# recursiveGecko/Formula-VAD

Hardware: AMD Instinct MI355X
Metric: 20ms audio frames/sec end-to-end VAD pipeline (higher is better)
Workload: dtype f32

## Files before the change

### formula-vad_amd/csrc/engine.cpp

```cpp
#include <algorithm>
#include <cctype>
#include <cmath>
#include <cstdio>
#include <cstdlib>
#include <cstring>
#include <atomic>
#include <mutex>
#include <thread>

#include "internal.h"

#ifndef FVAD_DIAG
#define FVAD_DIAG 0
#endif

namespace fvad {

int set_err(const fvad_ctx* ctx, int code, const std::string& msg)
{
    if (ctx) ctx->err = msg;
    return code;
}
int hip_fail(const fvad_ctx* ctx, hipError_t e, const char* what)
{
// ... 120 lines not shown
#endif
        tn.ws2_variant = (int)c;
    } else if (name == "ws2_waits") {
        long c = 0;
        if (!unset && (!to_long(c) || c < 0 || c > 0x7FFFFFFFL)) return FVAD_ERR_INVALID_ARGUMENT;
        tn.ws2_waits = (unsigned)c;
    } else if (name == "ws2_calibrate") {
        bool on = false;
        if (!to_bool(on)) return FVAD_ERR_INVALID_ARGUMENT;
        for (unsigned& w : tn.ws2_waits_cal) w = 0;
        if (on) { const int rc = calibrate_ws2_waits(ctx); if (rc) return rc; }
    } else if (name == "gru_lat_tiles") {
        long c = 0;
        if (!unset && (!to_long(c) || c < 1 || c > 3)) return FVAD_ERR_INVALID_ARGUMENT;
        tn.gru_lat_tiles = (int)c;
    } else if (name == "k4_plain_loads") { if (!to_bool(tn.k4_plain_loads)) return FVAD_ERR_INVALID_ARGUMENT; }
    else if (name == "no_pipeline") { if (!to_bool(tn.no_pipeline)) return FVAD_ERR_INVALID_ARGUMENT; }
    else if (name == "trace_run") { if (!to_bool(tn.trace_run)) return FVAD_ERR_INVALID_ARGUMENT; }
    else if (name == "run_groups") {
        if (!unset) {
            int sum = 0, n = 0, cur = 0;
            bool digit = false;
            for (char c : v + ",") {
                if (c >= '0' && c <= '9') { cur = cur * 10 + (c - '0'); digit = true; if (cur > 16) return FVAD_ERR_INVALID_ARGUMENT; }
                else if (c == ',' && digit && cur > 0) { sum += cur; ++n; cur = 0; digit = false; }
                else return FVAD_ERR_INVALID_ARGUMENT;
            }
            if (sum != 16 || n > 7) return FVAD_ERR_INVALID_ARGUMENT;
        }
        tn.run_groups = v;
// ... 659 lines not shown
```

### formula-vad_amd/csrc/internal.h

```cpp
#pragma once
#include <hip/hip_runtime.h>

#include <cstdint>
#include <map>
#include <memory>
#include <string>
#include <vector>

#include "../../include/fvad.h"
#include "kernels.h"

namespace fvad {

void hann_window_periodic(float* result, size_t n);
void hann_window_symmetric(float* result, size_t n);
float window_norm_factor(const float* w, size_t n);
void nsnet2_window(float* w320);
void make_twiddles(int n, std::vector<float>& out);
void make_super_twiddles(int ncfft, std::vector<float>& out);

struct HostWeights {
    int n_bins = 0, n_fc1 = 0, n_hidden = 0, n_fc2 = 0, n_fc3 = 0;
    std::vector<float> fc1_w, fc1_b, gru1_w, gru1_r, gru1_b, gru2_w, gru2_r, gru2_b, fc2_w, fc2_b,
        fc3_w, fc3_b, fc4_w, fc4_b;
// ... 111 lines not shown
    bool trace_run = false;
    std::string run_groups;
    int gru_lat_tiles = 0;
    bool k4_plain_loads = false;
    int copy_threads = 8;
    bool trace_kernels = false;
    bool reproducible = false;
    int vad_lane_map = 0;
    int vad_size_order = 0;
    int vad_chain = 0;
    int vad_avgs = 0;
    unsigned long long vad_avgs_max_bytes = 16ull << 30;
    int vad_trigger = 0;
    unsigned long long vad_trigger_max_bytes = 4ull << 30;
    int vad_seg_cap = 0;
    int ws2_variant = 0;
    unsigned ws2_waits = 0;
    unsigned ws2_waits_cal[4] = {0, 0, 0, 0};
    unsigned long long ws_spin_ticks = 0ull;
    bool ws_spin_auto = true;
};

}

struct fvad_ctx {
    int device = 0;
    int n_cu = 256;
    hipStream_t stream = nullptr;
    hipStream_t part_stream = nullptr;
    hipEvent_t part_ev = nullptr;
// ... 36 lines not shown
    } while (0)

int upload_model(fvad_ctx* ctx);
int dev_alloc(fvad_ctx* ctx, float** p, size_t n_floats, bool zero);
int grow(fvad_ctx* ctx, float** p, size_t* cap, size_t need);
void free_workspace_nn(Workspace& ws);
long planned_max_chunks(const fvad_ctx* ctx, long total, long max_chunks);
void plan_launches(const fvad_ctx* ctx, long total, long max_chunks, std::vector<long>& plan);
int ensure_workspace_plan(fvad_ctx* ctx, const std::vector<long>& plan);
long padded_batch(const fvad_ctx* ctx, long n, int T, int skip);
int nn_math_effective(const fvad_ctx* ctx);
int ensure_workspace(fvad_ctx* ctx, long n_chunks, int T, int skip, long n_last = 0);
int ensure_gru_ws(fvad_ctx* ctx);
int get_vad_plan(fvad_ctx* ctx, size_t n, VadFftPlan* out, bool force_generic = false);
bool fvad_fft_size_ok(size_t n);
int run_nn(fvad_ctx* ctx, long n_chunks_pad, int T, int skip, long n_real = 0);
int calibrate_ws2_waits(fvad_ctx* ctx);

struct LaneJob {
    const float* d_in;
    float* d_den;
    size_t n_chunks;
    LaneCarry* carry[2];
    int cur;
    float* d_rms;
    float* h_spec = nullptr;
    float* h_feat = nullptr;
    const int16_t* d_in16 = nullptr;
    int16_t* d_den16 = nullptr;
};
int run_chunks(fvad_ctx* ctx, std::vector<LaneJob>& jobs, long max_chunks, ChunkDesc* capture_descs = nullptr,
// ... 5 lines not shown
```

### formula-vad_amd/csrc/kernels.h

```cpp
#pragma once
#include <hip/hip_runtime.h>
#include <stddef.h>
#include <stdint.h>

#include "../../include/fvad.h"

enum { FVAD_ACT_NONE = 0, FVAD_ACT_RELU = 1, FVAD_ACT_SIGMOID = 2 };

constexpr int kNFft = 320;
constexpr int kNHop = 160;
constexpr int kFramesPerChunk = 50;
constexpr int kWarmupRows = 4;
constexpr int kRowsPerChunk = kFramesPerChunk + kWarmupRows;
constexpr int kNBins = 161;
constexpr int kFeatStride = 176;
constexpr int kDown = 3;
constexpr int kChunk48 = kFramesPerChunk * kNHop * kDown;
constexpr int kVadFft = 1024;
constexpr int kVadFftMax = 16384;

struct LaneCarry {
    float in_tail[kNHop * kDown];
    float feat_tail[kWarmupRows * kNBins];
    float ola_tail[kNHop];
// ... 39 lines not shown
};

int fvad_launch_panel_gemm(const float* A, int lda, const float* Wfrag, const float* bias, float* C,
                           int ldc, long rows, int nt, int n_blocks, int S_steps, int act,
                           int map_T, int map_skip, hipStream_t stream, int n_valid_tiles = 0,
                           const unsigned* guard = nullptr);
struct GemmRowMap {
    int n_rows = 0, L = 0, in_T = 0, in_t0 = 0, out_T = 0, out_t0 = 0;
};
int fvad_launch_panel_gemm_s_rows(const float* A, int lda, const float* Wfrag, const float* bias, float* C, int ldc,
                                  GemmRowMap rm, int nt, int n_blocks, int S_steps, int act, hipStream_t stream,
                                  int n_valid_tiles = 0, const unsigned* guard = nullptr);
int fvad_launch_panel_gemm_s(const float* A, int lda, const float* Wfrag, const float* bias, float* C, int ldc,
                             long rows, int nt, int n_blocks, int S_steps, int act, int map_T, int map_skip,
                             hipStream_t stream, int n_valid_tiles = 0, const unsigned* guard = nullptr);
int fvad_launch_panel_gemm3(const float* A, int lda, const float* Wfrag, const float* bias, float* C,
                            int ldc, long rows, int nt, int n_blocks, int S_steps, int K, int act,
                            int n_valid_tiles, int map_T, int map_skip, int n_wg, hipStream_t stream);
int fvad_launch_panel_gemm_h3(const float* A, int in_ts, int a_ld, const float* Wfrag, const float* bias, float* C,
                              int out, int c_ld, int seq_T, long row_tiles, int nt, int n_blocks, int K, int act,
                              int n_valid_tiles, int map_T, int map_skip, float sx, float sw, float out_sx, int n_wg,
                              hipStream_t stream);
int fvad_launch_gru_rec_h3(const float* gi, const float* Rfrag, const float* bR, float* hsplit,
                           long n_seq_pad, int T, int waves, float sx, float sw, hipStream_t stream);
int fvad_launch_gru_ws2_fallback(float* gi, const float* feat, const float* W1frag_nt2, const float* bG1, const float* R1frag, const float* bR1,
                                 const float* W2frag_nt2, const float* bW2, const float* R2frag, const float* bR2, float* h1, float* h2,
                                 long n_seq_pad, int T, unsigned* sync, unsigned long long* fallbacks, hipStream_t stream,
                                 int zero_at = 0, int zero_n = 0);
int fvad_launch_gru_lat(const float* gi, const float* R2frag, const float* bR, float* hout,
                        long n_seq_pad, int T, const unsigned* guard, int tile_major, hipStream_t stream, int row_tiles = 1);
void fvad_launch_zero_words(unsigned* p, int n, hipStream_t stream);
void fvad_launch_count_word(unsigned long long* counter, const unsigned* word, hipStream_t stream);
bool fvad_gru_ws_shape(long n_seq_pad, int n_cu, int* RT, int* G);
// ... 5 lines not shown
size_t fvad_gru_ws2_exchange_floats(long n_seq_pad);
bool fvad_gru_ws2_gi1_in_kernel(long n_seq_pad, int T, int n_cu, int variant);
bool fvad_gru_ws2_ok(long n_seq_pad, int T, int n_cu, int variant);
const char* fvad_gru_ws2_kernel_name(long n_seq_pad, int T, int n_cu, int variant);
int fvad_launch_gru_ws2(const float* gi1, const float* feat, const float* W1frag, const float* bG1, const float* R1frag, const float* bR1,
                        const float* W2frag, const float* bW2, const float* R2frag, const float* bR2, float* hout2, float* hx,
                        unsigned* flags, unsigned* err, long n_seq_pad, int T, int n_cu, unsigned long long spin_ticks, int variant,
                        unsigned waits, hipStream_t stream, unsigned* lsync = nullptr);
constexpr int kWs2LocalWords = 336;
bool fvad_gru_ws2_local_layer1(long n_seq_pad, int T, int n_cu, int variant);
int fvad_gru_ws2_wait_class(long n_seq_pad, int T, int n_cu, int variant);
unsigned fvad_gru_ws2_builtin_waits(int wait_class, bool local_layer1 = false);
int fvad_launch_gru_gen(const float* gi, int gi_ld, const float* R2frag, const float* bR, float* hout, int h_ld,
                        long n_seq_pad, int T, int J, hipStream_t stream);
int fvad_launch_gru_rec3(const float* gi, const float* R2frag, const float* bR, float* hout,
                         long n_seq_pad, int T, int waves, hipStream_t stream, float* hs3 = nullptr);
int fvad_launch_panel_gemm_b3(const float* A, int in_ts, int a_ld, const float* Wfrag, const float* bias, float* C,
                              int out, int c_ld, int seq_T, long row_tiles, int nt, int n_blocks, int K, int act,
                              int n_valid_tiles, int map_T, int map_skip, int n_wg, hipStream_t stream);

void fvad_launch_stft(const ChunkDesc* descs, int n_chunks, FftTables tb, float* feat,
                      float* spec, hipStream_t stream, int parts = 1);
void fvad_launch_istft(const ChunkDesc* descs, int n_chunks, FftTables tb, const float* spec,
                       const float* gains, int gains_rows_per_chunk, int gains_row0,
                       hipStream_t stream, int parts = 1);
void fvad_launch_vadfft(const float* den, long n_frames, VadFftPlan pl, int min_bin, int max_bin,
                        float* band_sum, float* bins_or_null, hipStream_t stream);
int fvad_launch_vadfft_jobs(const VadFftJob* jobs, int n_jobs, long max_frames, VadFftPlan pl,
                            int min_bin, int max_bin, hipStream_t stream, int any_bins, int n_cu, int plain_loads = 0);
constexpr int kVadBandsPerLaunch = 256;
struct VadBandSet {
// ... 162 lines not shown
```

### formula-vad_amd/csrc/kernels_nn.hip

```cpp

#include <hip/hip_runtime.h>
#include <stdint.h>
#include <type_traits>

#include "kernels.h"

#include "nn_device.h"

__device__ __forceinline__ float act_sigmoid(float x) { return 1.0f / (1.0f + expf(-x)); }

template <int NT, int ACT, int WAVES>
__global__ __launch_bounds__(WAVES * 64) void panel_gemm_kernel(
    const float* __restrict__ A, int lda, const float* __restrict__ Wfrag,
    const float* __restrict__ bias, float* __restrict__ C, int ldc, int S_steps, int row_map_T,
    int row_map_skip, int n_valid_tiles, const unsigned* guard)
{
    __shared__ __attribute__((aligned(16))) float slab[2][NT * 256];
    if (guard && *guard == 0) return;

    const int tid = threadIdx.x;
    const int lane = tid & 63;
    const int wave = tid >> 6;
    const int m = lane & 15;
    const int q = lane >> 4;
// ... 268 lines not shown
    }
};
template <int N> struct StaticFor<N, N> {
    template <class F> static __device__ __forceinline__ void run(F&&) {}
};

template <int OFF> __device__ __forceinline__ void lds_read_b128(f32x4& dst, unsigned addr)
{
    asm volatile("ds_read_b128 %0, %1 offset:%2" : "=v"(dst) : "v"(addr), "n"(OFF));
}
template <int N> __device__ __forceinline__ void lds_wait(f32x4& dst)
{
    asm volatile("s_waitcnt lgkmcnt(%1)" : "+v"(dst) : "n"(N));
}

template <int NT, int RT, int ACT, int SP, int WAVES>
__global__ __launch_bounds__(WAVES * 64) __attribute__((amdgpu_waves_per_eu(2, 2))) void panel_gemm3_kernel(
    const float* __restrict__ A, int lda, const float* __restrict__ Wfrag,
    const float* __restrict__ bias, float* __restrict__ C, int ldc, int S_steps, int n_blocks,
    int n_valid_tiles, int row_map_T, int row_map_skip, unsigned n_items, int tail_r)
{
    __shared__ __attribute__((aligned(16))) float slab[2][NT * SP * 256];
    __shared__ __attribute__((aligned(16))) float sbias[2][NT * 16];
    typedef __attribute__((address_space(3))) float lds_float;

    const int tid = threadIdx.x;
    const int lane = tid & 63;
    const int wave = __builtin_amdgcn_readfirstlane(tid >> 6);
    const int m = lane & 15;
    const int q = lane >> 4;
    const int P = (S_steps + SP - 1) / SP;
    constexpr int WAITN = (NT - 1 < 15) ? NT - 1 : 15;

    auto a_pointer = [&](unsigned item, int rt) -> const float* {
        const unsigned panel = item / (unsigned)n_blocks;
        const unsigned row = ((panel * WAVES + wave) * RT + rt) * 16 + m;
        unsigned a_row = row;
        if (row_map_T > 0) {
            const unsigned per = (unsigned)(row_map_T - row_map_skip);
            const unsigned qd = row / per;
            a_row = qd * (unsigned)row_map_T + (unsigned)row_map_skip + (row - qd * per);
        }
        return A + (size_t)a_row * (size_t)lda + 4 * q;
    };
    auto issue = [&](unsigned item, int p, float* dst) {
        const int nblk = (int)(item % (unsigned)n_blocks);
        const int s0 = p * SP;
        const int cnt = (S_steps - s0 < SP) ? (S_steps - s0) : SP;
        const float* src = Wfrag + ((size_t)nblk * S_steps + s0) * (NT * 256);
        const int nb = NT * cnt;
        constexpr int PER = (NT * SP + WAVES - 1) / WAVES;
#pragma unroll
        for (int i = 0; i < PER; ++i) {
            int b = wave + i * WAVES;
            b = b < nb ? b : nb - 1;
            __builtin_amdgcn_global_load_lds((const __attribute__((address_space(1))) void*)(src + b * 256 + lane * 4),
                                             (__attribute__((address_space(3))) void*)(dst + b * 256), 16, 0, 0);
        }
// ... 25 lines not shown
        const unsigned next_item = item + gridDim.x;
        const bool has_next = next_item < n_items;
        f32x4 acc[RT][NT];
        {
            const f32x4* bl = reinterpret_cast<const f32x4*>(sbias[bbuf]) + q;
#pragma unroll
            for (int t = 0; t < NT; ++t) {
                const f32x4 b4 = bl[4 * t];
#pragma unroll
                for (int rt = 0; rt < RT; ++rt) acc[rt][t] = b4;
            }
        }
        const float* a_nextitem[RT];
#pragma unroll
        for (int rt = 0; rt < RT; ++rt) a_nextitem[rt] = has_next ? a_pointer(next_item, rt) : a_ptr[rt];

        for (int p = 0; p < P; ++p) {
            const int s0 = p * SP;
            const int cnt = (S_steps - s0 < SP) ? (S_steps - s0) : SP;
            if (p + 1 < P) issue(item, p + 1, slab[buf ^ 1]);
            else if (has_next) { issue(next_item, 0, slab[buf ^ 1]); stage_bias(next_item, sbias[bbuf ^ 1]); }

            unsigned rd = slab_addr[buf];
            f32x4 w[NT];
            StaticFor<0, NT>::run([&](auto tc) {
                constexpr int t = decltype(tc)::value;
                lds_read_b128<t * 1024>(w[t], rd);
            });
            auto super_step = [&](int s, auto last_c) {
                constexpr bool LAST = decltype(last_c)::value;
// ... 17 lines not shown
                        for (int rt = 0; rt < RT; ++rt) acc[rt][t] = MFMA16(w[t].y, a0[rt].y, acc[rt][t]);
                    }
                    if (nr > 2) {
#pragma unroll
                        for (int rt = 0; rt < RT; ++rt) acc[rt][t] = MFMA16(w[t].z, a0[rt].z, acc[rt][t]);
                    }
                    if (nr > 3) {
#pragma unroll
                        for (int rt = 0; rt < RT; ++rt) acc[rt][t] = MFMA16(w[t].w, a0[rt].w, acc[rt][t]);
                    }
                };
                StaticFor<0, NT>::run([&](auto tc) {
                    constexpr int t = decltype(tc)::value;
                    if constexpr (LAST) {
                        lds_wait<((NT - 1 - t) < 15 ? (NT - 1 - t) : 15)>(w[t]);
                        mfmas(tc);
                    } else {
                        lds_wait<WAITN>(w[t]);
                        mfmas(tc);
                        lds_read_b128<(NT + t) * 1024>(w[t], rd);
                    }
                });
                rd += NT * 1024;
#pragma unroll
                for (int rt = 0; rt < RT; ++rt) a0[rt] = a1[rt];
            };
            for (int s = 0; s + 1 < cnt; ++s) super_step(s, std::false_type{});
            super_step(cnt - 1, std::true_type{});
            __syncthreads();
            buf ^= 1;
        }

#pragma unroll
        for (int rt = 0; rt < RT; ++rt) apre[rt] = *(gptr4)(a_nextitem[rt] + 16);
        const int nblk = (int)(item % (unsigned)n_blocks);
        const unsigned panel = item / (unsigned)n_blocks;
        const int bp_addr = ((lane >> 2) + 16 * (lane & 3)) * 4;
        float* c_ptr[RT];
#pragma unroll
        for (int rt = 0; rt < RT; ++rt) {
            const unsigned row = ((panel * WAVES + wave) * RT + rt) * 16 + (unsigned)(lane >> 2);
            c_ptr[rt] = C + (size_t)row * (size_t)ldc + nblk * (NT * 16) + 4 * (lane & 3);
        }
        const int valid_t = n_valid_tiles - nblk * NT;
        auto emit = [&](int t, int rt) {
            f32x4 v = acc[rt][t];
            if (ACT == FVAD_ACT_RELU) {
                v.x = fmaxf(v.x, 0.f); v.y = fmaxf(v.y, 0.f); v.z = fmaxf(v.z, 0.f); v.w = fmaxf(v.w, 0.f);
            } else if (ACT == FVAD_ACT_SIGMOID) {
                v.x = act_sigmoid(v.x); v.y = act_sigmoid(v.y); v.z = act_sigmoid(v.z); v.w = act_sigmoid(v.w);
            }
            f32x4 o;
            o.x = __int_as_float(__builtin_amdgcn_ds_bpermute(bp_addr, __float_as_int(v[0])));
            o.y = __int_as_float(__builtin_amdgcn_ds_bpermute(bp_addr, __float_as_int(v[1])));
            o.z = __int_as_float(__builtin_amdgcn_ds_bpermute(bp_addr, __float_as_int(v[2])));
            o.w = __int_as_float(__builtin_amdgcn_ds_bpermute(bp_addr, __float_as_int(v[3])));
// ... 9 lines not shown
            for (int t = 0; t < NT; ++t) {
                if (t < valid_t) {
#pragma unroll
                    for (int rt = 0; rt < RT; ++rt) emit(t, rt);
                }
            }
        }
        bbuf ^= 1;
#pragma unroll
        for (int rt = 0; rt < RT; ++rt) a_ptr[rt] = a_nextitem[rt];
    }
}

int fvad_launch_panel_gemm3(const float* A, int lda, const float* Wfrag, const float* bias, float* C,
                            int ldc, long rows, int nt, int n_blocks, int S_steps, int K, int act,
                            int n_valid_tiles, int map_T, int map_skip, int n_wg, hipStream_t stream)
{
    if (rows % 256) return -1;
    const int n_last = K - 16 * (S_steps - 1);
    const int tail_r = n_last >= 4 ? 4 : (n_last < 1 ? 4 : n_last);
    const unsigned n_items = (unsigned)((rows / 256) * n_blocks);
    const unsigned grid = n_items < (unsigned)n_wg ? n_items : (unsigned)n_wg;
#define CASE3(NT_, ACT_, SP_)                                                                         \
    if (nt == NT_ && act == ACT_) {                                                                   \
        hipLaunchKernelGGL((panel_gemm3_kernel<NT_, 2, ACT_, SP_, 8>), dim3(grid), dim3(512), 0, stream, \
                           A, lda, Wfrag, bias, C, ldc, S_steps, n_blocks, n_valid_tiles, map_T,      \
                           map_skip, n_items, tail_r);                                                \
        return 0;                                                                                     \
    }
    CASE3(15, FVAD_ACT_NONE, 5)
    CASE3(13, FVAD_ACT_RELU, 5)
    CASE3(11, FVAD_ACT_SIGMOID, 6)
#undef CASE3
    return -1;
}


template <int WAVES>
__device__ __forceinline__ void gru3_issue_slab(const float* __restrict__ src, float* lds_dst, int wave, unsigned lane16)
{
    asm volatile("" : "+v"(lane16));
#pragma unroll
    for (int b = wave; b < 3 * GRU_J; b += WAVES) {
        __builtin_amdgcn_global_load_lds(
            (const __attribute__((address_space(1))) void*)((const __attribute__((address_space(1))) char*)src + b * 1024 + lane16),
            (__attribute__((address_space(3))) void*)(lds_dst + b * 256), 16, 0, 0);
    }
}

template <int WAVES, int D, bool TS3>
__global__ __launch_bounds__(WAVES * 64) void gru_rec3_kernel(const float* __restrict__ gi,
                                                              const float* __restrict__ R2frag,
                                                              const float* __restrict__ bR,
                                                              float* hout, int T, float* hs3)
{
    __shared__ __attribute__((aligned(16))) float slab[2][GRU2_SLAB];
    typedef __attribute__((address_space(3))) float lds_float;

    const int tid = threadIdx.x;
    const int lane = tid & 63;
    const int wave = __builtin_amdgcn_readfirstlane(tid >> 6);
    const int m = lane & 15;
    const int q = lane >> 4;
    typedef const __attribute__((address_space(1))) char* gbytes;
    const size_t seq0 = (size_t)(blockIdx.x * WAVES + wave) * 16;
    gbytes gi_w = (gbytes)(gi + seq0 * T * (3 * GRU_H));
    __attribute__((address_space(1))) char* h_w = (__attribute__((address_space(1))) char*)(hout + seq0 * T * GRU_H);
    gbytes bR_b = (gbytes)bR;
    const unsigned gi_off = ((unsigned)m * (unsigned)T * (3 * GRU_H) + 4u * q) * 4u;
    const unsigned h_off = ((unsigned)m * (unsigned)T * GRU_H + 4u * q) * 4u;
    const unsigned b_off = 16u * q;
    auto ld4 = [](gbytes base, unsigned off) {
        asm volatile("" : "+v"(off));
        return *(const __attribute__((address_space(1))) f32x4*)(base + off);
    };
    const unsigned slab_addr[2] = {(unsigned)(uintptr_t)(lds_float*)slab[0] + (unsigned)lane * 16u,
                                   (unsigned)(uintptr_t)(lds_float*)slab[1] + (unsigned)lane * 16u};
    __attribute__((address_space(1))) char* hs_w = nullptr;
    if (TS3) hs_w = (__attribute__((address_space(1))) char*)(hs3 + (size_t)(blockIdx.x * WAVES + wave) * T * (13 * 768));
    auto store_split3 = [&](__attribute__((address_space(1))) char* hs_t, int J, const f32x4& h) {
        typedef __bf16 b16x4 __attribute__((ext_vector_type(4)));
        typedef __bf16 b16x8 __attribute__((ext_vector_type(8)));
        b16x4 ph, pm, pl;
#pragma unroll
// ... 29 lines not shown
        f32x4 h;
#pragma unroll
        for (int r = 0; r < 4; ++r) {
            const float z = fast_sigmoid(giz[r]);
            const float rr = fast_sigmoid(gir[r]);
            const float n = fast_tanh(gin[r] + rr * bn[r]);
            h[r] = (1.0f - z) * n + z * 0.0f;
        }
        *(__attribute__((address_space(1))) f32x4*)(h_w + 64 * J + h_off) = h;
        if (TS3) store_split3(hs_w, J, h);
    }
    __syncthreads();
    int buf = 0;

    for (int t = 1; t < T; ++t) {
        gbytes gi_t = gi_w + (size_t)t * (12 * GRU_H);
        gbytes h_prev = (gbytes)h_w + (size_t)(t - 1) * (4 * GRU_H);
        __attribute__((address_space(1))) char* h_out = h_w + (size_t)t * (4 * GRU_H);

        f32x4 hreg[GRU_J];
#pragma unroll
        for (int S = 0; S < GRU_J; ++S) hreg[S] = ld4(h_prev + 64 * S, h_off);
#pragma unroll
        for (int S = 0; S < GRU_J; ++S) asm volatile("" : "+v"(hreg[S]));

        for (int J = 0; J < GRU_J; ++J) {
            const int nJ = (J + 1 == GRU_J) ? 0 : J + 1;
            gru3_issue_slab<WAVES>(R2frag + (size_t)nJ * GRU2_SLAB, slab[buf ^ 1], wave, (unsigned)lane * 16u);

            const unsigned rdz = slab_addr[buf], rdr = rdz + GRU_J * 1024, rdn = rdz + 2 * GRU_J * 1024;
// ... 440 lines not shown
    }
}

int fvad_launch_gru_gen(const float* gi, int gi_ld, const float* R2frag, const float* bR, float* hout, int h_ld,
                        long n_seq_pad, int T, int J, hipStream_t stream)
{
    if (n_seq_pad % 16 || J < 1 || J > 64) return -1;
    const size_t lds = (size_t)2 * J * 1024;
    if (lds > 48 * 1024 &&
        hipFuncSetAttribute((const void*)gru_gen_kernel, hipFuncAttributeMaxDynamicSharedMemorySize, (int)lds) != hipSuccess) return -2;
    hipLaunchKernelGGL(gru_gen_kernel, dim3((unsigned)(n_seq_pad / 16)), dim3(512), lds, stream, gi, gi_ld, R2frag, bR, hout, h_ld, T, J);
    return 0;
}

int fvad_launch_gru_rec3(const float* gi, const float* R2frag, const float* bR, float* hout,
                         long n_seq_pad, int T, int waves, hipStream_t stream, float* hs3)
{
#define REC3(W_)                                                                                                          \
    if (waves == W_) {                                                                                                    \
        if (hs3) hipLaunchKernelGGL((gru_rec3_kernel<W_, 2, true>), dim3((unsigned)(n_seq_pad / (16 * W_))), dim3(64 * W_), 0, stream, gi, R2frag, bR, hout, T, hs3); \
        else hipLaunchKernelGGL((gru_rec3_kernel<W_, 2, false>), dim3((unsigned)(n_seq_pad / (16 * W_))), dim3(64 * W_), 0, stream, gi, R2frag, bR, hout, T, hs3); \
        return 0;                                                                                                         \
    }
    REC3(12)
    REC3(8)
    REC3(4)
#undef REC3
    return -1;
}
```

### formula-vad_amd/csrc/nn_dispatch.cpp

```cpp
#include <algorithm>
#include <atomic>
#include <cmath>
#include <cstdio>
#include <cstdlib>
#include <cstring>
#include <mutex>
#include <thread>

#include "internal.h"

namespace fvad {

void free_workspace_nn(Workspace& ws)
{
    float** bufs[] = {&ws.feat, &ws.spec, &ws.a1, &ws.gi, &ws.h1, &ws.h2, &ws.hs1, &ws.hs2, &ws.f2, &ws.f3, &ws.gains};
    for (float** b : bufs) { if (*b) hipFree(*b); *b = nullptr; }
    if (ws.descs) hipFree(ws.descs);
    if (ws.h_descs) hipHostFree(ws.h_descs);
    ws.descs = nullptr; ws.h_descs = nullptr;
    ws.descs_mirror.clear();
    ws.cap_chunks = 0;
    ws.cap_rows = 0;
    ws.a1_cap_rows = ws.h_cap_rows = ws.hs_cap_rows = 0;
}
// ... 310 lines not shown
    time_end(ctx);
    time_begin(ctx, "fc2_gemm");
    rc |= fvad_launch_panel_gemm(ws.h2, g.Hp, m.g_fc2_w.p, m.g_fc2_b.p, ws.f2, g.N2p, rows_out, 8, g.N2p / 128, g.J, FVAD_ACT_RELU, skip ? T : 0, skip, st);
    time_end(ctx);
    time_begin(ctx, "fc3_gemm");
    rc |= fvad_launch_panel_gemm(ws.f2, g.N2p, m.g_fc3_w.p, m.g_fc3_b.p, ws.f3, g.N3p, rows_out, 8, g.N3p / 128, S(g.N2), FVAD_ACT_RELU, 0, 0, st);
    time_end(ctx);
    time_begin(ctx, "fc4_gemm");
    rc |= fvad_launch_panel_gemm(ws.f3, g.N3p, m.g_fc4_w.p, m.g_fc4_b.p, ws.gains, kFeatStride, rows_out, 11, 1, S(g.N3), FVAD_ACT_SIGMOID, 0, 0, st);
    time_end(ctx);
    if (rc) return set_err(ctx, FVAD_ERR_INVALID_ARGUMENT, "no kernel instance for this layer shape");
    FVAD_HIP(ctx, hipGetLastError());
    return FVAD_OK;
}

int run_nn(fvad_ctx* ctx, long n_pad, int T, int skip, long n_real)
{
    if (!ctx->dm.loaded) return set_err(ctx, FVAD_ERR_NO_MODEL, "NSNet2 weights not loaded");
    if (n_real <= 0 || n_real > n_pad) n_real = n_pad;
    if (ctx->dm.generic) return run_nn_generic(ctx, n_pad, T, skip);
    Workspace& ws = ctx->ws;
    const DeviceModel& m = ctx->dm;
    hipStream_t st = ctx->stream;
    const long rows = n_pad * T;
    const long rows_out = n_pad * (T - skip);
    int rc = 0;
    const Tuning& tn = ctx->tune;
    const char* force = tn.gemm_kernel.empty() ? nullptr : tn.gemm_kernel.c_str();
    const int math = nn_math_effective(ctx);
    const bool h3 = math == FVAD_NN_MATH_F16X3, b3 = math == FVAD_NN_MATH_BF16X3;
    if ((h3 || b3) && n_pad % 128) return set_err(ctx, FVAD_ERR_INVALID_ARGUMENT, "the emulated kernels need a batch padded to 128 sequences");
// ... 31 lines not shown
        rc |= gemm_b3(ws.b3_f2, 1, 19, m.fc3_b3, m.fc3h3_b.p, ws.b3_f3, 2, 19, T - skip, G * (T - skip), 10, 4, 600, FVAD_ACT_RELU, 38, 0, 0);
        time_end(ctx);
        time_begin(ctx, "fc4_gemm");
        rc |= gemm_b3(ws.b3_f3, 1, 19, m.fc4_b3, m.fc4h3_b.p, ws.gains, 0, kFeatStride, T - skip, G * (T - skip), 12, 1, 600, FVAD_ACT_SIGMOID, 11, 0, 0);
        time_end(ctx);
        if (rc) return set_err(ctx, FVAD_ERR_INVALID_ARGUMENT, "no kernel instance for this layer shape");
        FVAD_HIP(ctx, hipGetLastError());
        return FVAD_OK;
    }
    const bool big = h3 || (force ? force[1] != '1' : (tn.reproducible || n_pad >= 2048));
    if (tn.reproducible && !force && (rows % 256 || rows_out % 256))
        return set_err(ctx, FVAD_ERR_INVALID_ARGUMENT, "reproducible: batch not padded to the persistent GEMM's 256-row panels");
    if (big && rows % 256 == 0 && rows_out % 256 == 0) {
        auto gemm = [&](const float* A, int lda, const float* W, const float* b, float* Cc, int ldc, long r, int nt,
                        int nblk, int S, int K, int act, int valid, int mT, int mskip) {
            return fvad_launch_panel_gemm3(A, lda, W, b, Cc, ldc, r, nt, nblk, S, K, act, valid, mT, mskip, ctx->n_cu, st);
        };
        auto gemm_h3 = [&](const float* A, int in_ts, int a_ld, const DevBuf& W, const DeviceModel::H3Scale& sc, const float* b,
                           float* Cc, int out, int c_ld, int seq_T, long row_tiles, int nt, int nblk, int K, int act,
                           int valid, int mT, int mskip, float out_sx) {
            return fvad_launch_panel_gemm_h3(A, in_ts, a_ld, W.p, b, Cc, out, c_ld, seq_T, row_tiles, nt, nblk, K, act, valid,
                                             mT, mskip, sc.sx, sc.sw, out_sx, ctx->n_cu, st);
        };
        if (h3) {
            int waves = n_pad % 192 == 0 ? 12 : 8;
            if ((tn.h3_waves == 8 || tn.h3_waves == 12) && n_pad % (16 * tn.h3_waves) == 0) waves = tn.h3_waves;
            ctx->last_nn_path = std::string("f16x3: panel_gemm_h3 + gru_rec_h3<") + std::to_string(waves) + ">";
            const long G = n_pad / 16;
            time_begin(ctx, "gru1_in_gemm_fc1folded");
            rc |= gemm_h3(ws.feat, 0, kFeatStride, m.gi1f_h3, m.h3_gi1f, m.gi1f_bzr.p, ws.gi, 1, 75, T, G * T, 15, 5, 161, FVAD_ACT_NONE, 75, 0, 0, 1.0f);
            time_end(ctx);
// ... 13 lines not shown
            rc |= gemm_h3(ws.f2, 1, 19, m.fc3_h3, m.h3_fc3, m.fc3h3_b.p, ws.f3, 2, 19, T - skip, G * (T - skip), 10, 4, 600, FVAD_ACT_RELU, 38, 0, 0, m.h3_fc4.sx);
            time_end(ctx);
            time_begin(ctx, "fc4_gemm");
            rc |= gemm_h3(ws.f3, 1, 19, m.fc4_h3, m.h3_fc4, m.fc4h3_b.p, ws.gains, 0, kFeatStride, T - skip, G * (T - skip), 12, 1, 600, FVAD_ACT_SIGMOID, 11, 0, 0, 1.0f);
            time_end(ctx);
            if (rc) return set_err(ctx, FVAD_ERR_INVALID_ARGUMENT, "no kernel instance for this layer shape");
            FVAD_HIP(ctx, hipGetLastError());
            return FVAD_OK;
        }
        const bool fold = !(force && strstr(force, "nofold"));
        const GruChoice gc = pick_gru(ctx, n_pad, T, fold);
        ctx->last_nn_path = std::string("f32: panel_gemm3") + (fold ? " (fc1 folded)" : "") + " + " +
                            (gc.version == 3 ? "gru_rec3<" + std::to_string(gc.waves) + ">" : gc.version == 5 ? std::string("gru_ws") : std::string("gru_lat"));
        if (gc.version == 5 && (rc = prepare_gru_ws(ctx, n_pad))) return rc;
        const bool bzr = gc.version == 3;
        if (fold) {
            time_begin(ctx, "gru1_in_gemm_fc1folded");
            rc |= gemm(ws.feat, kFeatStride, m.gi1f_w.p, bzr ? m.gi1f_bzr.p : m.gi1f_b.p, ws.gi, 1200, rows, 15, 5, 11, 161, FVAD_ACT_NONE, 75, 0, 0);
            time_end(ctx);
        } else {
            time_begin(ctx, "fc1_gemm");
            rc |= fvad_launch_panel_gemm(ws.feat, kFeatStride, m.fc1_w.p, m.fc1_b.p, ws.a1, 400, rows, 25, 1, 11, FVAD_ACT_NONE, 0, 0, st);
            time_end(ctx);
            time_begin(ctx, "gru1_in_gemm");
            rc |= gemm(ws.a1, 400, m.gi1v2_w.p, m.gi1_btm.p, ws.gi, 1200, rows, 15, 5, 25, 400, FVAD_ACT_NONE, 75, 0, 0);
            time_end(ctx);
        }
        time_begin(ctx, "gru1_rec");
        rc |= launch_gru(ctx, gc, ws.gi, m.r1v2, m.br1.p, ws.h1, n_pad, T, 0, 1);
        time_end(ctx);
        time_begin(ctx, "gru2_in_gemm");
        rc |= gemm(ws.h1, 400, m.gi2v2_w.p, bzr ? m.gi2_bzr.p : m.gi2_btm.p, ws.gi, 1200, rows, 15, 5, 25, 400, FVAD_ACT_NONE, 75, 0, 0);
        time_end(ctx);
        time_begin(ctx, "gru2_rec");
        rc |= launch_gru(ctx, gc, ws.gi, m.r2v2, m.br2.p, ws.h2, n_pad, T, 1, 1);
        time_end(ctx);
        time_begin(ctx, "fc2_gemm");
        rc |= gemm(ws.h2, 400, m.fc2v3_w.p, m.fc2v3_b.p, ws.f2, 608, rows_out, 13, 3, 25, 400, FVAD_ACT_RELU, 38, skip ? T : 0, skip);
        time_end(ctx);
        time_begin(ctx, "fc3_gemm");
        rc |= gemm(ws.f2, 608, m.fc3v3_w.p, m.fc3v3_b.p, ws.f3, 608, rows_out, 13, 3, 38, 600, FVAD_ACT_RELU, 38, 0, 0);
        time_end(ctx);
        time_begin(ctx, "fc4_gemm");
        rc |= gemm(ws.f3, 608, m.fc4_w.p, m.fc4_b.p, ws.gains, kFeatStride, rows_out, 11, 1, 38, 600, FVAD_ACT_SIGMOID, 11, 0, 0);
// ... 208 lines not shown
    long total = 0;
    for (auto& j : jobs) total += (long)j.n_chunks;
    if (total == 0) return FVAD_OK;
    std::vector<long> plan;
    plan_launches(ctx, total, max_chunks, plan);
    int rc = ensure_workspace_plan(ctx, plan);
    if (rc) return rc;
    Workspace& ws = ctx->ws;
    size_t launch_i = 0;

    size_t job = 0, chunk_in_job = 0;
    while (job < jobs.size()) {
        const long cap = std::min<long>(launch_i < plan.size() ? plan[launch_i] : plan.back(), ws.cap_chunks);
        ++launch_i;
        long n = 0;
        std::vector<size_t> touched;
        struct Tap { size_t job, chunk0, count; long batch0; };
        std::vector<Tap> taps;
        const int slot = ws.desc_slot;
        ChunkDesc* hd;
        if (capture_descs) hd = capture_descs + capture_off;
        else {
            ws.desc_slot ^= 1;
            FVAD_HIP(ctx, hipEventSynchronize(ws.desc_ev[slot]));
            hd = ws.h_descs + (size_t)slot * (size_t)ws.cap_chunks;
        }
        size_t j = job, c = chunk_in_job;
        while (j < jobs.size() && n < cap) {
            LaneJob& lj = jobs[j];
            if (lj.n_chunks == 0) { ++j; c = 0; continue; }
            const size_t take = std::min<size_t>(lj.n_chunks - c, (size_t)(cap - n));
            if (lj.h_spec || lj.h_feat) taps.push_back({j, c, take, n});
            for (size_t k = 0; k < take; ++k) {
                ChunkDesc& d = hd[n + (long)k];
                d.in = lj.d_in ? lj.d_in + (c + k) * (size_t)kChunk48 : nullptr;
                d.in16 = lj.d_in16 ? lj.d_in16 + (c + k) * (size_t)kChunk48 : nullptr;
                d.den = lj.d_den + (c + k) * (size_t)kChunk48;
                d.den16 = lj.d_den16 ? lj.d_den16 + (c + k) * (size_t)kChunk48 : nullptr;
                d.carry_in = lj.carry[lj.cur];
                d.carry_out = lj.carry[lj.cur ^ 1];
                d.first = (k == 0);
                d.last = (k + 1 == take);
                d.rms = lj.d_rms ? lj.d_rms + (c + k) : nullptr;
            }
            touched.push_back(j);
            n += (long)take;
// ... 11 lines not shown
        const int fft_parts = n <= 85 ? 3 : (n <= 128 ? 2 : 1);
        fvad_launch_stft(dd, (int)n, ctx->tb, ws.feat, ws.spec, ctx->stream, fft_parts);
        time_end(ctx);
        for (const Tap& t : taps) {
            const LaneJob& lj = jobs[t.job];
            if (lj.h_spec)
                FVAD_HIP(ctx, hipMemcpyAsync(lj.h_spec + t.chunk0 * (size_t)(kFramesPerChunk * kNBins * 2),
                                             ws.spec + (size_t)t.batch0 * (kFramesPerChunk * kNBins * 2),
                                             t.count * (size_t)(kFramesPerChunk * kNBins * 2) * sizeof(float), hipMemcpyDeviceToHost, ctx->stream));
            if (lj.h_feat)
                FVAD_HIP(ctx, hipMemcpy2DAsync(lj.h_feat + t.chunk0 * (size_t)(kRowsPerChunk * kNBins), kNBins * sizeof(float),
                                               ws.feat + (size_t)t.batch0 * (kRowsPerChunk * kFeatStride), kFeatStride * sizeof(float),
                                               kNBins * sizeof(float), t.count * (size_t)kRowsPerChunk, hipMemcpyDeviceToHost, ctx->stream));
        }
        const long n_pad = padded_batch(ctx, n, kRowsPerChunk, kWarmupRows);
        rc = run_nn(ctx, n_pad, kRowsPerChunk, kWarmupRows, n);
        if (rc) return rc;
        time_begin(ctx, "istft320_ola_up3");
        fvad_launch_istft(dd, (int)n, ctx->tb, ws.spec, ws.gains, kFramesPerChunk, 0, ctx->stream, fft_parts);
        time_end(ctx);
        for (size_t t : touched) jobs[t].cur ^= 1;
        if (n_launches) ++*n_launches;
        job = j;
        chunk_in_job = c;
    }
    FVAD_HIP(ctx, hipGetLastError());
    return FVAD_OK;
}

}
```

Measured before the change: 25.06 million.

## Skip redundant warmup-row GRU input GEMM and trim padded MFMA tiles

Adds an nn_trim tunable, on by default, with two parts. The first computes the folded GRU1 input GEMM only for each chunk's own rows plus the warmup rows of each lane's first chunk, using a compacted row map. The GRU recurrence then reads warmup-row inputs from the previous chunk's rows, which are the same frames, instead of recomputing them. The second makes the ReLU panel GEMM skip MFMAs for the padded last tile. This removes duplicated GEMM work on overlapping warmup frames, at the cost of an extra launch and more complex addressing that relies on chunks of a lane being contiguous.

```diff
diff --git a/formula-vad_amd/csrc/engine.cpp b/formula-vad_amd/csrc/engine.cpp
--- a/formula-vad_amd/csrc/engine.cpp
+++ b/formula-vad_amd/csrc/engine.cpp
@@ -158,6 +158,12 @@
         long c = 0;
         if (!unset && (!to_long(c) || c < 1 || c > 3)) return FVAD_ERR_INVALID_ARGUMENT;
         tn.gru_lat_tiles = (int)c;
+    } else if (name == "nn_trim") {
+        if (unset || v == "all") tn.nn_trim = 3;
+        else if (v == "tiles") tn.nn_trim = 1;
+        else if (v == "rows") tn.nn_trim = 2;
+        else if (v == "none") tn.nn_trim = 0;
+        else return FVAD_ERR_INVALID_ARGUMENT;
     } else if (name == "k4_plain_loads") { if (!to_bool(tn.k4_plain_loads)) return FVAD_ERR_INVALID_ARGUMENT; }
     else if (name == "no_pipeline") { if (!to_bool(tn.no_pipeline)) return FVAD_ERR_INVALID_ARGUMENT; }
     else if (name == "trace_run") { if (!to_bool(tn.trace_run)) return FVAD_ERR_INVALID_ARGUMENT; }
diff --git a/formula-vad_amd/csrc/internal.h b/formula-vad_amd/csrc/internal.h
--- a/formula-vad_amd/csrc/internal.h
+++ b/formula-vad_amd/csrc/internal.h
@@ -149,6 +149,7 @@
     int vad_trigger = 0;
     unsigned long long vad_trigger_max_bytes = 4ull << 30;
     int vad_seg_cap = 0;
+    int nn_trim = 3;
     int ws2_variant = 0;
     unsigned ws2_waits = 0;
     unsigned ws2_waits_cal[4] = {0, 0, 0, 0};
@@ -215,7 +216,11 @@
 int ensure_gru_ws(fvad_ctx* ctx);
 int get_vad_plan(fvad_ctx* ctx, size_t n, VadFftPlan* out, bool force_generic = false);
 bool fvad_fft_size_ok(size_t n);
-int run_nn(fvad_ctx* ctx, long n_chunks_pad, int T, int skip, long n_real = 0);
+struct NnLanes {
+    const ChunkDesc* descs = nullptr;
+    long n_lanes = 0, chunks_per_lane = 0;
+};
+int run_nn(fvad_ctx* ctx, long n_chunks_pad, int T, int skip, long n_real = 0, const NnLanes* lanes = nullptr);
 int calibrate_ws2_waits(fvad_ctx* ctx);
 
 struct LaneJob {
diff --git a/formula-vad_amd/csrc/kernels.h b/formula-vad_amd/csrc/kernels.h
--- a/formula-vad_amd/csrc/kernels.h
+++ b/formula-vad_amd/csrc/kernels.h
@@ -77,9 +77,14 @@
 int fvad_launch_panel_gemm_s(const float* A, int lda, const float* Wfrag, const float* bias, float* C, int ldc,
                              long rows, int nt, int n_blocks, int S_steps, int act, int map_T, int map_skip,
                              hipStream_t stream, int n_valid_tiles = 0, const unsigned* guard = nullptr);
+struct Gemm3RowMap {
+    int per = 0, T = 0, skip = 0;
+    long n_q = 0;
+};
 int fvad_launch_panel_gemm3(const float* A, int lda, const float* Wfrag, const float* bias, float* C,
                             int ldc, long rows, int nt, int n_blocks, int S_steps, int K, int act,
-                            int n_valid_tiles, int map_T, int map_skip, int n_wg, hipStream_t stream);
+                            int n_valid_tiles, int map_T, int map_skip, int n_wg, hipStream_t stream, bool trim_tiles = false,
+                            const Gemm3RowMap* cmap = nullptr);
 int fvad_launch_panel_gemm_h3(const float* A, int in_ts, int a_ld, const float* Wfrag, const float* bias, float* C,
                               int out, int c_ld, int seq_T, long row_tiles, int nt, int n_blocks, int K, int act,
                               int n_valid_tiles, int map_T, int map_skip, float sx, float sw, float out_sx, int n_wg,
@@ -115,7 +120,8 @@
 int fvad_launch_gru_gen(const float* gi, int gi_ld, const float* R2frag, const float* bR, float* hout, int h_ld,
                         long n_seq_pad, int T, int J, hipStream_t stream);
 int fvad_launch_gru_rec3(const float* gi, const float* R2frag, const float* bR, float* hout,
-                         long n_seq_pad, int T, int waves, hipStream_t stream, float* hs3 = nullptr);
+                         long n_seq_pad, int T, int waves, hipStream_t stream, float* hs3 = nullptr,
+                         const ChunkDesc* first_of = nullptr, long n_real = 0);
 int fvad_launch_panel_gemm_b3(const float* A, int in_ts, int a_ld, const float* Wfrag, const float* bias, float* C,
                               int out, int c_ld, int seq_T, long row_tiles, int nt, int n_blocks, int K, int act,
                               int n_valid_tiles, int map_T, int map_skip, int n_wg, hipStream_t stream);
diff --git a/formula-vad_amd/csrc/kernels_nn.hip b/formula-vad_amd/csrc/kernels_nn.hip
--- a/formula-vad_amd/csrc/kernels_nn.hip
+++ b/formula-vad_amd/csrc/kernels_nn.hip
@@ -306,11 +306,12 @@
     asm volatile("s_waitcnt lgkmcnt(%1)" : "+v"(dst) : "n"(N));
 }
 
-template <int NT, int RT, int ACT, int SP, int WAVES>
+template <int NT, int RT, int ACT, int SP, int WAVES, bool CMAP = false, bool TRIMT = false>
 __global__ __launch_bounds__(WAVES * 64) __attribute__((amdgpu_waves_per_eu(2, 2))) void panel_gemm3_kernel(
     const float* __restrict__ A, int lda, const float* __restrict__ Wfrag,
     const float* __restrict__ bias, float* __restrict__ C, int ldc, int S_steps, int n_blocks,
-    int n_valid_tiles, int row_map_T, int row_map_skip, unsigned n_items, int tail_r)
+    int n_valid_tiles, int row_map_T, int row_map_skip, unsigned n_items, int tail_r, int row_map_per,
+    unsigned row_map_qmax, int n_mfma_tiles)
 {
     __shared__ __attribute__((aligned(16))) float slab[2][NT * SP * 256];
     __shared__ __attribute__((aligned(16))) float sbias[2][NT * 16];
@@ -324,16 +325,18 @@
     const int P = (S_steps + SP - 1) / SP;
     constexpr int WAITN = (NT - 1 < 15) ? NT - 1 : 15;
 
+    auto map_row = [&](unsigned row) -> unsigned {
+        if (row_map_T <= 0) return row;
+        const unsigned per = (unsigned)row_map_per;
+        unsigned qd = row / per;
+        const unsigned tt = row - qd * per;
+        if (CMAP) qd = qd < row_map_qmax ? qd : row_map_qmax;
+        return qd * (unsigned)row_map_T + (unsigned)row_map_skip + tt;
+    };
     auto a_pointer = [&](unsigned item, int rt) -> const float* {
         const unsigned panel = item / (unsigned)n_blocks;
         const unsigned row = ((panel * WAVES + wave) * RT + rt) * 16 + m;
-        unsigned a_row = row;
-        if (row_map_T > 0) {
-            const unsigned per = (unsigned)(row_map_T - row_map_skip);
-            const unsigned qd = row / per;
-            a_row = qd * (unsigned)row_map_T + (unsigned)row_map_skip + (row - qd * per);
-        }
-        return A + (size_t)a_row * (size_t)lda + 4 * q;
+        return A + (size_t)map_row(row) * (size_t)lda + 4 * q;
     };
     auto issue = [&](unsigned item, int p, float* dst) {
         const int nblk = (int)(item % (unsigned)n_blocks);
@@ -389,6 +392,7 @@
         const float* a_nextitem[RT];
 #pragma unroll
         for (int rt = 0; rt < RT; ++rt) a_nextitem[rt] = has_next ? a_pointer(next_item, rt) : a_ptr[rt];
+        const bool skip_last = TRIMT && n_mfma_tiles - (int)(item % (unsigned)n_blocks) * NT < NT;
 
         for (int p = 0; p < P; ++p) {
             const int s0 = p * SP;
@@ -436,10 +440,10 @@
                     constexpr int t = decltype(tc)::value;
                     if constexpr (LAST) {
                         lds_wait<((NT - 1 - t) < 15 ? (NT - 1 - t) : 15)>(w[t]);
-                        mfmas(tc);
+                        if (!(TRIMT && t == NT - 1 && skip_last)) mfmas(tc);
                     } else {
                         lds_wait<WAITN>(w[t]);
-                        mfmas(tc);
+                        if (!(TRIMT && t == NT - 1 && skip_last)) mfmas(tc);
                         lds_read_b128<(NT + t) * 1024>(w[t], rd);
                     }
                 });
@@ -461,7 +465,8 @@
         float* c_ptr[RT];
 #pragma unroll
         for (int rt = 0; rt < RT; ++rt) {
-            const unsigned row = ((panel * WAVES + wave) * RT + rt) * 16 + (unsigned)(lane >> 2);
+            unsigned row = ((panel * WAVES + wave) * RT + rt) * 16 + (unsigned)(lane >> 2);
+            if (CMAP) row = map_row(row);
             c_ptr[rt] = C + (size_t)row * (size_t)ldc + nblk * (NT * 16) + 4 * (lane & 3);
         }
         const int valid_t = n_valid_tiles - nblk * NT;
@@ -501,23 +506,32 @@
 
 int fvad_launch_panel_gemm3(const float* A, int lda, const float* Wfrag, const float* bias, float* C,
                             int ldc, long rows, int nt, int n_blocks, int S_steps, int K, int act,
-                            int n_valid_tiles, int map_T, int map_skip, int n_wg, hipStream_t stream)
+                            int n_valid_tiles, int map_T, int map_skip, int n_wg, hipStream_t stream, bool trim_tiles,
+                            const Gemm3RowMap* cmap)
 {
     if (rows % 256) return -1;
+    int map_per = map_T - map_skip;
+    unsigned map_qmax = 0;
+    if (cmap) {
+        if (cmap->per <= 0 || cmap->T < cmap->skip + cmap->per || cmap->skip < 0 || cmap->n_q <= 0 || rows < cmap->n_q * (long)cmap->per) return -1;
+        map_T = cmap->T; map_skip = cmap->skip; map_per = cmap->per; map_qmax = (unsigned)(cmap->n_q - 1);
+    }
+    const int n_mfma_tiles = trim_tiles ? n_valid_tiles : nt * n_blocks;
     const int n_last = K - 16 * (S_steps - 1);
     const int tail_r = n_last >= 4 ? 4 : (n_last < 1 ? 4 : n_last);
     const unsigned n_items = (unsigned)((rows / 256) * n_blocks);
     const unsigned grid = n_items < (unsigned)n_wg ? n_items : (unsigned)n_wg;
-#define CASE3(NT_, ACT_, SP_)                                                                         \
-    if (nt == NT_ && act == ACT_) {                                                                   \
-        hipLaunchKernelGGL((panel_gemm3_kernel<NT_, 2, ACT_, SP_, 8>), dim3(grid), dim3(512), 0, stream, \
+#define CASE3(NT_, ACT_, SP_, CMAP_, TRIMT_)                                                          \
+    if (nt == NT_ && act == ACT_ && (cmap != nullptr) == CMAP_) {                                     \
+        hipLaunchKernelGGL((panel_gemm3_kernel<NT_, 2, ACT_, SP_, 8, CMAP_, TRIMT_>), dim3(grid), dim3(512), 0, stream, \
                            A, lda, Wfrag, bias, C, ldc, S_steps, n_blocks, n_valid_tiles, map_T,      \
-                           map_skip, n_items, tail_r);                                                \
+                           map_skip, n_items, tail_r, map_per, map_qmax, n_mfma_tiles);               \
         return 0;                                                                                     \
     }
-    CASE3(15, FVAD_ACT_NONE, 5)
-    CASE3(13, FVAD_ACT_RELU, 5)
-    CASE3(11, FVAD_ACT_SIGMOID, 6)
+    CASE3(15, FVAD_ACT_NONE, 5, false, false)
+    CASE3(15, FVAD_ACT_NONE, 5, true, false)
+    CASE3(13, FVAD_ACT_RELU, 5, false, true)
+    CASE3(11, FVAD_ACT_SIGMOID, 6, false, false)
 #undef CASE3
     return -1;
 }
@@ -539,7 +553,8 @@
 __global__ __launch_bounds__(WAVES * 64) void gru_rec3_kernel(const float* __restrict__ gi,
                                                               const float* __restrict__ R2frag,
                                                               const float* __restrict__ bR,
-                                                              float* hout, int T, float* hs3)
+                                                              float* hout, int T, float* hs3,
+                                                              const ChunkDesc* __restrict__ descs, unsigned n_real)
 {
     __shared__ __attribute__((aligned(16))) float slab[2][GRU2_SLAB];
     typedef __attribute__((address_space(3))) float lds_float;
@@ -551,10 +566,16 @@
     const int q = lane >> 4;
     typedef const __attribute__((address_space(1))) char* gbytes;
     const size_t seq0 = (size_t)(blockIdx.x * WAVES + wave) * 16;
-    gbytes gi_w = (gbytes)(gi + seq0 * T * (3 * GRU_H));
+    gbytes gi_w = (gbytes)(gi + seq0 * T * (3 * GRU_H)) - (size_t)kWarmupRows * (3 * GRU_H) * 4;
     __attribute__((address_space(1))) char* h_w = (__attribute__((address_space(1))) char*)(hout + seq0 * T * GRU_H);
     gbytes bR_b = (gbytes)bR;
-    const unsigned gi_off = ((unsigned)m * (unsigned)T * (3 * GRU_H) + 4u * q) * 4u;
+    constexpr unsigned GI_SHIFT = kWarmupRows * (3 * GRU_H) * 4u;
+    const unsigned gi_off_own = ((unsigned)m * (unsigned)T * (3 * GRU_H) + 4u * q) * 4u + GI_SHIFT;
+    unsigned gi_off = gi_off_own;
+    if (descs) {
+        const unsigned seq = (unsigned)seq0 + (unsigned)m;
+        if (seq >= n_real || !descs[seq].first) gi_off -= GI_SHIFT;
+    }
     const unsigned h_off = ((unsigned)m * (unsigned)T * GRU_H + 4u * q) * 4u;
     const unsigned b_off = 16u * q;
     auto ld4 = [](gbytes base, unsigned off) {
@@ -614,6 +635,7 @@
     int buf = 0;
 
     for (int t = 1; t < T; ++t) {
+        if (t == kWarmupRows) gi_off = gi_off_own;
         gbytes gi_t = gi_w + (size_t)t * (12 * GRU_H);
         gbytes h_prev = (gbytes)h_w + (size_t)(t - 1) * (4 * GRU_H);
         __attribute__((address_space(1))) char* h_out = h_w + (size_t)t * (4 * GRU_H);
@@ -1084,12 +1106,13 @@
 }
 
 int fvad_launch_gru_rec3(const float* gi, const float* R2frag, const float* bR, float* hout,
-                         long n_seq_pad, int T, int waves, hipStream_t stream, float* hs3)
-{
+                         long n_seq_pad, int T, int waves, hipStream_t stream, float* hs3, const ChunkDesc* first_of, long n_real)
+{
+    if (first_of && (T <= kWarmupRows || n_real < 1 || n_real > n_seq_pad)) return -1;
 #define REC3(W_)                                                                                                          \
     if (waves == W_) {                                                                                                    \
-        if (hs3) hipLaunchKernelGGL((gru_rec3_kernel<W_, 2, true>), dim3((unsigned)(n_seq_pad / (16 * W_))), dim3(64 * W_), 0, stream, gi, R2frag, bR, hout, T, hs3); \
-        else hipLaunchKernelGGL((gru_rec3_kernel<W_, 2, false>), dim3((unsigned)(n_seq_pad / (16 * W_))), dim3(64 * W_), 0, stream, gi, R2frag, bR, hout, T, hs3); \
+        if (hs3) hipLaunchKernelGGL((gru_rec3_kernel<W_, 2, true>), dim3((unsigned)(n_seq_pad / (16 * W_))), dim3(64 * W_), 0, stream, gi, R2frag, bR, hout, T, hs3, first_of, (unsigned)n_real); \
+        else hipLaunchKernelGGL((gru_rec3_kernel<W_, 2, false>), dim3((unsigned)(n_seq_pad / (16 * W_))), dim3(64 * W_), 0, stream, gi, R2frag, bR, hout, T, hs3, first_of, (unsigned)n_real); \
         return 0;                                                                                                         \
     }
     REC3(12)
diff --git a/formula-vad_amd/csrc/nn_dispatch.cpp b/formula-vad_amd/csrc/nn_dispatch.cpp
--- a/formula-vad_amd/csrc/nn_dispatch.cpp
+++ b/formula-vad_amd/csrc/nn_dispatch.cpp
@@ -348,7 +348,7 @@
     return FVAD_OK;
 }
 
-int run_nn(fvad_ctx* ctx, long n_pad, int T, int skip, long n_real)
+int run_nn(fvad_ctx* ctx, long n_pad, int T, int skip, long n_real, const NnLanes* lanes)
 {
     if (!ctx->dm.loaded) return set_err(ctx, FVAD_ERR_NO_MODEL, "NSNet2 weights not loaded");
     if (n_real <= 0 || n_real > n_pad) n_real = n_pad;
@@ -410,7 +410,7 @@
     if (big && rows % 256 == 0 && rows_out % 256 == 0) {
         auto gemm = [&](const float* A, int lda, const float* W, const float* b, float* Cc, int ldc, long r, int nt,
                         int nblk, int S, int K, int act, int valid, int mT, int mskip) {
-            return fvad_launch_panel_gemm3(A, lda, W, b, Cc, ldc, r, nt, nblk, S, K, act, valid, mT, mskip, ctx->n_cu, st);
+            return fvad_launch_panel_gemm3(A, lda, W, b, Cc, ldc, r, nt, nblk, S, K, act, valid, mT, mskip, ctx->n_cu, st, (tn.nn_trim & 1) != 0);
         };
         auto gemm_h3 = [&](const float* A, int in_ts, int a_ld, const DevBuf& W, const DeviceModel::H3Scale& sc, const float* b,
                            float* Cc, int out, int c_ld, int seq_T, long row_tiles, int nt, int nblk, int K, int act,
@@ -454,7 +454,22 @@
                             (gc.version == 3 ? "gru_rec3<" + std::to_string(gc.waves) + ">" : gc.version == 5 ? std::string("gru_ws") : std::string("gru_lat"));
         if (gc.version == 5 && (rc = prepare_gru_ws(ctx, n_pad))) return rc;
         const bool bzr = gc.version == 3;
-        if (fold) {
+        const bool trim_rows = (tn.nn_trim & 2) && fold && gc.version == 3 && lanes && lanes->descs && lanes->chunks_per_lane > 0 &&
+                               lanes->n_lanes * lanes->chunks_per_lane == n_real && T == kRowsPerChunk && skip == kWarmupRows &&
+                               (n_pad * (T - skip)) % 256 == 0;
+        if (trim_rows) ctx->last_nn_path += ", gi1 rows 4..53";
+        if (trim_rows) {
+            Gemm3RowMap own, first;
+            own.per = T - skip; own.T = T; own.skip = skip; own.n_q = n_pad;
+            first.per = skip; first.T = (int)(lanes->chunks_per_lane * T); first.skip = 0; first.n_q = lanes->n_lanes;
+            const long first_rows = (lanes->n_lanes * skip + 255) / 256 * 256;
+            time_begin(ctx, "gru1_in_gemm_fc1folded");
+            rc |= fvad_launch_panel_gemm3(ws.feat, kFeatStride, m.gi1f_w.p, m.gi1f_bzr.p, ws.gi, 1200, n_pad * (T - skip), 15, 5, 11, 161, FVAD_ACT_NONE, 75,
+                                          0, 0, ctx->n_cu, st, false, &own);
+            rc |= fvad_launch_panel_gemm3(ws.feat, kFeatStride, m.gi1f_w.p, m.gi1f_bzr.p, ws.gi, 1200, first_rows, 15, 5, 11, 161, FVAD_ACT_NONE, 75,
+                                          0, 0, ctx->n_cu, st, false, &first);
+            time_end(ctx);
+        } else if (fold) {
             time_begin(ctx, "gru1_in_gemm_fc1folded");
             rc |= gemm(ws.feat, kFeatStride, m.gi1f_w.p, bzr ? m.gi1f_bzr.p : m.gi1f_b.p, ws.gi, 1200, rows, 15, 5, 11, 161, FVAD_ACT_NONE, 75, 0, 0);
             time_end(ctx);
@@ -467,7 +482,8 @@
             time_end(ctx);
         }
         time_begin(ctx, "gru1_rec");
-        rc |= launch_gru(ctx, gc, ws.gi, m.r1v2, m.br1.p, ws.h1, n_pad, T, 0, 1);
+        if (trim_rows) rc |= (n_pad % (16 * gc.waves)) ? -1 : fvad_launch_gru_rec3(ws.gi, m.r1v2.p, m.br1.p, ws.h1, n_pad, T, gc.waves, st, nullptr, lanes->descs, n_real);
+        else rc |= launch_gru(ctx, gc, ws.gi, m.r1v2, m.br1.p, ws.h1, n_pad, T, 0, 1);
         time_end(ctx);
         time_begin(ctx, "gru2_in_gemm");
         rc |= gemm(ws.h1, 400, m.gi2v2_w.p, bzr ? m.gi2_bzr.p : m.gi2_btm.p, ws.gi, 1200, rows, 15, 5, 25, 400, FVAD_ACT_NONE, 75, 0, 0);
@@ -706,6 +722,7 @@
         const long cap = std::min<long>(launch_i < plan.size() ? plan[launch_i] : plan.back(), ws.cap_chunks);
         ++launch_i;
         long n = 0;
+        NnLanes nl;
         std::vector<size_t> touched;
         struct Tap { size_t job, chunk0, count; long batch0; };
         std::vector<Tap> taps;
@@ -722,6 +739,8 @@
             LaneJob& lj = jobs[j];
             if (lj.n_chunks == 0) { ++j; c = 0; continue; }
             const size_t take = std::min<size_t>(lj.n_chunks - c, (size_t)(cap - n));
+            if (nl.n_lanes++ == 0) nl.chunks_per_lane = (long)take;
+            else if (nl.chunks_per_lane != (long)take) nl.chunks_per_lane = 0;
             if (lj.h_spec || lj.h_feat) taps.push_back({j, c, take, n});
             for (size_t k = 0; k < take; ++k) {
                 ChunkDesc& d = hd[n + (long)k];
@@ -763,7 +782,8 @@
                                                kNBins * sizeof(float), t.count * (size_t)kRowsPerChunk, hipMemcpyDeviceToHost, ctx->stream));
         }
         const long n_pad = padded_batch(ctx, n, kRowsPerChunk, kWarmupRows);
-        rc = run_nn(ctx, n_pad, kRowsPerChunk, kWarmupRows, n);
+        nl.descs = dd;
+        rc = run_nn(ctx, n_pad, kRowsPerChunk, kWarmupRows, n, &nl);
         if (rc) return rc;
         time_begin(ctx, "istft320_ola_up3");
         fvad_launch_istft(dd, (int)n, ctx->tb, ws.spec, ws.gains, kFramesPerChunk, 0, ctx->stream, fft_parts);
```

After: 25.35 million (median of 6 runs). 1.01x the previous value.
